# kevalmorabia97/CoVA-Web-Object-Detection

Measured on AMD Instinct MI355X. Metric: webpages/sec fwd+bwd (90 bboxes, K=24), higher is better.
Workload: dtype f32

## Files before the change

cova-web-object-detection_amd/csrc/bn1d.hip:

```cpp
#include "bn_tail.h"

namespace {

constexpr int COLS = 8, SLICES = 128, RUN = 32;
constexpr int THREADS = COLS * SLICES;

__device__ __forceinline__ void slices_total(double (*s_a)[COLS], double (*s_b)[COLS], int tx, int ty, double a, double b,
                                             double &ta, double &tb)
{
    s_a[ty][tx] = a;
    s_b[ty][tx] = b;
    __syncthreads();
    ta = 0.0;
    tb = 0.0;
    if (ty == 0)
        for (int j = 0; j < SLICES; ++j) {
            ta += s_a[j][tx];
            tb += s_b[j][tx];
        }
}

template <bool DROP>
__global__ __launch_bounds__(THREADS) void bn1d_fwd_kernel(
    const float *__restrict__ x, int ldx, int R, int C, const float *__restrict__ gamma, const float *__restrict__ beta,
// ... 213 lines not shown
    const float *__restrict__ invstd, const float *__restrict__ scale, int R, int C, float *__restrict__ dgamma,
    float *__restrict__ dbeta, float *__restrict__ dz, int lddz, float *__restrict__ dz_colsum)
{
    __shared__ double s_red[V4_THREADS / 64][V4_COLS][2];
    __shared__ float s_c1[V4_COLS], s_c2[V4_COLS];
    const int q = threadIdx.x & 1, slice = threadIdx.x >> 1, lane = threadIdx.x & 63, wave = threadIdx.x >> 6;
    const int c = blockIdx.x * V4_COLS + q * 4;
    const bool colok = c < C;
    const float inv = DROP ? 1.f / (1.f - p) : 1.f;
    float mu[4] = {0.f, 0.f, 0.f, 0.f}, is[4] = {0.f, 0.f, 0.f, 0.f}, sc[4] = {0.f, 0.f, 0.f, 0.f};
    if (colok) {
#pragma unroll
        for (int j = 0; j < 4; ++j) { mu[j] = mean[c + j]; is[j] = invstd[c + j]; sc[j] = scale[c + j]; }
    }
    float4 gv[NR], av[NR], zv[NR];
    uchar4 mv[NR];
#pragma unroll
    for (int u = 0; u < NR; ++u) {
        const int r = slice + u * V4_SLICES;
        const bool ok = colok && r < R;
        const size_t rr = ok ? (size_t)r : 0;
        const int cc = ok ? c : 0;
        gv[u] = *reinterpret_cast<const float4 *>(dout + rr * ldg + cc);
        zv[u] = *reinterpret_cast<const float4 *>(z + rr * ldz + cc);
        if (act != nullptr) av[u] = *reinterpret_cast<const float4 *>(act + rr * lda + cc);
        if (DROP) mv[u] = *reinterpret_cast<const uchar4 *>(drop_mask + rr * C + cc);
        if (!ok) gv[u] = make_float4(0.f, 0.f, 0.f, 0.f);
    }
    double v[4][2] = {{0.0, 0.0}, {0.0, 0.0}, {0.0, 0.0}, {0.0, 0.0}};
    float dy[NR][4], xh[NR][4];
#pragma unroll
    for (int u = 0; u < NR; ++u) {
        const float g4[4] = {gv[u].x, gv[u].y, gv[u].z, gv[u].w};
        const float z4[4] = {zv[u].x, zv[u].y, zv[u].z, zv[u].w};
        const float a4[4] = {av[u].x, av[u].y, av[u].z, av[u].w};
        const uint8_t m4[4] = {mv[u].x, mv[u].y, mv[u].z, mv[u].w};
#pragma unroll
        for (int j = 0; j < 4; ++j) {
            float g = g4[j];
            if (DROP) g = m4[j] ? g * inv : 0.f;
            if (act != nullptr && !(a4[j] > 0.f)) g = 0.f;
            dy[u][j] = g;
            xh[u][j] = (z4[j] - mu[j]) * is[j];
            v[j][0] += (double)g;
            v[j][1] = fma((double)g, (double)xh[u][j], v[j][1]);
        }
    }
    double ta, tb;
    v4_totals(s_red, v, q, lane, wave, ta, tb);
    const int cf = blockIdx.x * V4_COLS + threadIdx.x;
    if (threadIdx.x < V4_COLS && cf < C) {
        if (dbeta) dbeta[cf] = (float)ta;
        if (dgamma) dgamma[cf] = (float)tb;
        s_c1[threadIdx.x] = (float)(ta / (double)R);
        s_c2[threadIdx.x] = (float)(tb / (double)R);
    }
    __syncthreads();
    double cs[4][2] = {{0.0, 0.0}, {0.0, 0.0}, {0.0, 0.0}, {0.0, 0.0}};
    if (colok) {
        float s[4] = {0.f, 0.f, 0.f, 0.f};
#pragma unroll
        for (int u = 0; u < NR; ++u) {
            const int r = slice + u * V4_SLICES;
            if (r >= R) break;
            float o[4];
#pragma unroll
            for (int j = 0; j < 4; ++j) {
                o[j] = sc[j] * (dy[u][j] - s_c1[q * 4 + j] - xh[u][j] * s_c2[q * 4 + j]);
                s[j] += o[j];
            }
            *reinterpret_cast<float4 *>(dz + (size_t)r * lddz + c) = make_float4(o[0], o[1], o[2], o[3]);
        }
#pragma unroll
        for (int j = 0; j < 4; ++j) cs[j][0] = (double)s[j];
    }
    if (dz_colsum != nullptr) {
        __syncthreads();
        double t1, t2;
        v4_totals(s_red, cs, q, lane, wave, t1, t2);
        if (threadIdx.x < V4_COLS && cf < C) dz_colsum[cf] = (float)t1;
    }
}

int g_bn1d_variant = 1;

inline bool al16(const void *p) { return ((uintptr_t)p & 15) == 0; }

}

int cova_internal_set_bn1d_variant(int v) { g_bn1d_variant = v; return COVA_OK; }
int cova_internal_get_bn1d_variant() { return (int)g_bn1d_variant; }

COVA_API int cova_bn1d_fwd(const float *x, int ldx, int R, int C, const float *gamma, const float *beta,
                           float *running_mean, float *running_var, long long *num_batches_tracked, float momentum,
                           float eps, int relu, float *out, int ldo, float *dropped, int ld_dropped, uint8_t *mask,
                           float p, unsigned long long seed, int mask_given, float *scale, float *shift, float *mean,
                           float *invstd, void *stream)
{
    COVA_REQUIRE(x && gamma && beta && out && scale && shift && mean && invstd && R > 0 && C > 0);
    COVA_REQUIRE((running_mean == nullptr) == (running_var == nullptr));
    COVA_REQUIRE(dropped == nullptr || (mask != nullptr && p >= 0.f && p < 1.f));
    const bool v4 = g_bn1d_variant != 0 && C % 4 == 0 && ldx % 4 == 0 && ldo % 4 == 0 && al16(x) && al16(out) &&
                    (dropped == nullptr || (ld_dropped % 4 == 0 && al16(dropped) && ((uintptr_t)mask & 3) == 0)) &&
                    R <= 8 * V4_SLICES;
    if (v4) {
        const dim3 g4(cdiv(C, V4_COLS));
#define BN1D_FWD_V4(NR_, DROP_)                                                                                             \
        hipLaunchKernelGGL((bn1d_fwd_v4_kernel<NR_, DROP_>), g4, dim3(V4_THREADS), 0, (hipStream_t)stream, x, ldx, R, C, gamma, \
                           beta, running_mean, running_var, num_batches_tracked, momentum, eps, relu, out, ldo, dropped,   \
                           ld_dropped, mask, p, seed, mask_given, scale, shift, mean, invstd)
        if (R <= 3 * V4_SLICES) { if (dropped) BN1D_FWD_V4(3, true); else BN1D_FWD_V4(3, false); }
        else if (R <= 6 * V4_SLICES) { if (dropped) BN1D_FWD_V4(6, true); else BN1D_FWD_V4(6, false); }
        else { if (dropped) BN1D_FWD_V4(8, true); else BN1D_FWD_V4(8, false); }
#undef BN1D_FWD_V4
        COVA_LAUNCH_CHECK();
        return COVA_OK;
    }
    const dim3 grid(cdiv(C, COLS));
    if (dropped)
        hipLaunchKernelGGL(bn1d_fwd_kernel<true>, grid, dim3(THREADS), 0, (hipStream_t)stream, x, ldx, R, C, gamma, beta,
                           running_mean, running_var, num_batches_tracked, momentum, eps, relu, out, ldo, dropped,
                           ld_dropped, mask, p, seed, mask_given, scale, shift, mean, invstd);
    else
        hipLaunchKernelGGL(bn1d_fwd_kernel<false>, grid, dim3(THREADS), 0, (hipStream_t)stream, x, ldx, R, C, gamma, beta,
                           running_mean, running_var, num_batches_tracked, momentum, eps, relu, out, ldo, dropped,
                           ld_dropped, mask, p, seed, mask_given, scale, shift, mean, invstd);
    COVA_LAUNCH_CHECK();
    return COVA_OK;
}

COVA_API int cova_bn1d_bwd(const float *dout, int ldg, const uint8_t *drop_mask, float p, const float *act, int lda,
                           const float *z, int ldz, const float *mean, const float *invstd, const float *scale, int R,
                           int C, float *dgamma, float *dbeta, float *dz, int lddz, float *dz_colsum, void *stream)
{
    COVA_REQUIRE(dout && z && mean && invstd && scale && dz && R > 0 && C > 0);
    COVA_REQUIRE(drop_mask == nullptr || (p >= 0.f && p < 1.f));
    const bool v4 = g_bn1d_variant != 0 && C % 4 == 0 && ldg % 4 == 0 && ldz % 4 == 0 && lddz % 4 == 0 && al16(dout) &&
                    al16(z) && al16(dz) && (act == nullptr || (lda % 4 == 0 && al16(act))) &&
                    (drop_mask == nullptr || ((uintptr_t)drop_mask & 3) == 0) && R <= 6 * V4_SLICES;
    if (v4) {
        const dim3 g4(cdiv(C, V4_COLS));
#define BN1D_BWD_V4(NR_, DROP_)                                                                                             \
        hipLaunchKernelGGL((bn1d_bwd_v4_kernel<NR_, DROP_>), g4, dim3(V4_THREADS), 0, (hipStream_t)stream, dout, ldg, drop_mask, \
                           p, act, lda, z, ldz, mean, invstd, scale, R, C, dgamma, dbeta, dz, lddz, dz_colsum)
        if (R <= 3 * V4_SLICES) { if (drop_mask) BN1D_BWD_V4(3, true); else BN1D_BWD_V4(3, false); }
        else { if (drop_mask) BN1D_BWD_V4(6, true); else BN1D_BWD_V4(6, false); }
#undef BN1D_BWD_V4
        COVA_LAUNCH_CHECK();
        return COVA_OK;
    }
    const dim3 grid(cdiv(C, COLS));
    if (drop_mask)
        hipLaunchKernelGGL(bn1d_bwd_kernel<true>, grid, dim3(THREADS), 0, (hipStream_t)stream, dout, ldg, drop_mask, p, act,
                           lda, z, ldz, mean, invstd, scale, R, C, dgamma, dbeta, dz, lddz, dz_colsum);
    else
        hipLaunchKernelGGL(bn1d_bwd_kernel<false>, grid, dim3(THREADS), 0, (hipStream_t)stream, dout, ldg, drop_mask, p, act,
                           lda, z, ldz, mean, invstd, scale, R, C, dgamma, dbeta, dz, lddz, dz_colsum);
    COVA_LAUNCH_CHECK();
    return COVA_OK;
}
```

cova-web-object-detection_amd/engine.py:

```python
import ctypes
import os

import torch

from . import _lib
from .weights import BACKBONE_CHANNELS as C64

GAT_MAX_K = 1024

call, query = _lib.call, _lib.query
BN_MOMENTUM, BN_EPS, LEAKY_SLOPE = 0.1, 1e-5, 0.2


DROPOUT_KEYS = ("decoder.0", "decoder.3")


def is_train(training, key):
    if isinstance(training, bool):
        return training
    if hasattr(training, "get"):
        return bool(training.get(key, True))
    return bool(training)


# ... 212 lines not shown
    st = bn_state(C, like, count, training)
    g, b = params[prefix + "weight"], params[prefix + "bias"]
    rm, rv = buffers[prefix + "running_mean"], buffers[prefix + "running_var"]
    if training:
        upd = update_running
        partial, nparts = fold_partials(partial, nparts, 2 * C)
        if STAT_SYNC is not None:
            partial, nparts, count = _global_stats(partial, nparts, 2 * C, count, unit)
            st.count = float(count)
        nbt = buffers.get(prefix + "num_batches_tracked") if upd else None
        call("cova_bn_finalize_fwd", partial, nparts, C, float(count), g, b, rm if upd else None,
             rv if upd else None, nbt, BN_MOMENTUM, BN_EPS, st.scale, st.shift, st.mean, st.invstd)
    else:
        call("cova_bn_eval_params", g, b, rm, rv, BN_EPS, C, st.scale, st.shift, st.mean, st.invstd)
    return st


def colstats(x, ld, R, C):
    n = query("cova_colreduce_num_chunks", R, C)
    part = _empty((n, 2, C), x)
    call("cova_colstats", x, ld, R, C, part)
    return part, n


def bn_backward(dout, ldd, act, lda, z, ldz, st, R, dz, lddz, dres=None, lddres=0, gout=None,
                prefix=None, unit="boxes", drop=None, colsum=None):
    C = st.C
    if (bn1d_fused(not st.frozen) and dres is None and R > 0 and z.dim() == 2 and dz.data_ptr() != dout.data_ptr()):
        dgamma = _gbuf(gout, (prefix or "") + "weight", (C,), z)
        dbeta = _gbuf(gout, (prefix or "") + "bias", (C,), z)
        call("cova_bn1d_bwd", dout, ldd, drop[0] if drop else None, float(drop[1]) if drop else 0.0, act, lda, z, ldz,
             st.mean, st.invstd, st.scale, R, C, dgamma, dbeta, dz, lddz, colsum)
        return dgamma, dbeta
    if drop is not None:
        dy = _empty((R, C), dout)
        call("cova_dropout_bwd", dout, ldd, drop[0], dy, C, R, C, float(drop[1]))
        dout, ldd = dy, C
    n = query("cova_colreduce_num_chunks", R, C)
    part = _empty((n, 2, C), z)
    call("cova_bn_bwd_reduce", dout, ldd, act, lda, z, ldz, st.mean, st.invstd, R, C, part)
    dgamma = _gbuf(gout, (prefix or "") + "weight", (C,), z)
    dbeta = _gbuf(gout, (prefix or "") + "bias", (C,), z)
    coef = bn_finalize_bwd(part, n, C, R, dgamma, dbeta, unit, frozen=st.frozen)
    call("cova_bn_bwd_apply", dout, ldd, act, lda, z, ldz, st.mean, st.invstd, st.scale, coef, dz,
         lddz, dres, lddres, R, C)
    if colsum is not None:
        call("cova_colsum", dz, lddz, R, C, colsum)
    return dgamma, dbeta


class _BnTailStruct(ctypes.Structure):
    _fields_ = [("mode", ctypes.c_int), ("counter", ctypes.c_void_p), ("count", ctypes.c_double),
                ("gamma", ctypes.c_void_p), ("beta", ctypes.c_void_p), ("running_mean", ctypes.c_void_p),
                ("running_var", ctypes.c_void_p), ("num_batches_tracked", ctypes.c_void_p),
                ("momentum", ctypes.c_float), ("eps", ctypes.c_float), ("scale", ctypes.c_void_p),
                ("shift", ctypes.c_void_p), ("mean", ctypes.c_void_p), ("invstd", ctypes.c_void_p),
                ("dgamma", ctypes.c_void_p), ("dbeta", ctypes.c_void_p), ("abc", ctypes.c_void_p)]


class BnTail:
    _COUNTERS = {}

    def __init__(self, mode, like, count, **ptrs):
        key = (like.device, torch.cuda.current_stream(like.device).cuda_stream)
        ctr = BnTail._COUNTERS.get(key)
        if ctr is None:
            ctr = BnTail._COUNTERS[key] = torch.zeros((1,), dtype=torch.int32, device=like.device)
        self.keep = [ctr] + [v for v in ptrs.values() if isinstance(v, torch.Tensor)]
        c = _BnTailStruct()
        c.mode, c.counter, c.count = mode, ctr.data_ptr(), float(count)
        c.momentum, c.eps = BN_MOMENTUM, BN_EPS
        for k, v in ptrs.items():
            setattr(c, k, v.data_ptr() if isinstance(v, torch.Tensor) else None)
        self.c = c

    @property
    def ptr(self):
        return ctypes.addressof(self.c)


class Options:
    overlap_allreduce = os.environ.get("COVA_OVERLAP_ALLREDUCE", "1") != "0"
    bn_tail = os.environ.get("COVA_BN_TAIL", "1") != "0"


OPTIONS = Options()

CONV3_KEYS = ["convnet.4.0.conv1", "convnet.4.0.conv2", "convnet.4.1.conv1", "convnet.4.1.conv2"]
BN3_KEYS = ["convnet.4.0.bn1.", "convnet.4.0.bn2.", "convnet.4.1.bn1.", "convnet.4.1.bn2."]


class LazyFeature:
    __slots__ = ("z", "x", "scale", "shift", "shape")

    def __init__(self, z, x, scale, shift):
        self.z, self.x, self.scale, self.shift, self.shape = z, x, scale, shift, tuple(z.shape)


def is_bottleneck(params):
    return "convnet.4.0.conv3.weight" in params


@on_device_of(0)
def convstack_fwd(images, params, buffers, training, save=True, lazy_out=False):
    _check(images)
    B, _, H, W = images.shape
    H1, W1 = query("cova_conv_out_size", H, 7, 2, 3), query("cova_conv_out_size", W, 7, 2, 3)
    H2, W2 = query("cova_conv_out_size", H1, 3, 2, 1), query("cova_conv_out_size", W1, 3, 2, 1)
    bottleneck = is_bottleneck(params)
    layer2 = has_layer2(params)
    lazy_out = lazy_out and not layer2
    sv = {"images": images, "dims": (B, H, W, H1, W1, H2, W2), "kind": "bottleneck" if bottleneck else "basic"}
    if bottleneck:
        sv["_w3"] = conv3_weights([params["convnet.4.%d.conv2.weight" % b] for b in (0, 1, 2)], images)
    else:
        sv["_w3"] = conv3_weights([params[k + ".weight"] for k in CONV3_KEYS], images)
    y1 = _empty((B, H1, W1, C64), images)
    nt1 = query("cova_conv1_num_partials", B, H, W)
    stem_train = is_train(training, "convnet.1.")
    part = _empty((nt1, 2, C64), images) if stem_train else None
    if stem_train and tails_on():
        bn1, tail = bn_tail_fwd("convnet.1.", params, buffers, C64, images, B * H1 * W1)
        call("cova_conv1_fwd_tail", images, params["convnet.0.weight"], y1, part, B, H, W, tail.ptr)
    else:
        call("cova_conv1_fwd_tail", images, params["convnet.0.weight"], y1, part, B, H, W, None)
        bn1 = bn_params("convnet.1.", params, buffers, C64, images, training, part, nt1, B * H1 * W1, unit="pages")
    p1 = _empty((B, H2, W2, C64), images)
    idx = _empty((B, H2, W2, C64), images, torch.uint8)
    want_ymax = save and (stem_train or bottleneck)
    ymax = _empty((B, H2, W2, C64), images) if want_ymax else None
    call("cova_bn_relu_maxpool_fwd", y1, bn1.scale, bn1.shift, p1, idx, ymax, B, H1, W1)
    sv.update(y1=y1, bn1=bn1, idx=idx, ymax=ymax)
    if bottleneck:
        feat = _layer1_bottleneck_fwd(p1, params, buffers, training, save, lazy_out, sv)
    else:
        feat = _layer1_basic_fwd(p1, params, buffers, training, save, lazy_out, sv)
    if layer2:
        feat = _layer2_fwd(feat, params, buffers, training, save, sv)
    return feat, (sv if save else None)


def conv3_num_partials(B, H, W):
    return query("cova_conv3x3_wino4_num_partials", B, H, W)


def conv3x3_pro(u, inp, in2, abc, relu, addend, act, msc, msh, z, mean, invstd, out, part, B, H, W, tail=None,
                act_bits=None):
    if tail is not None:
        if act_bits is not None:
            act = None
        call("cova_conv3x3_wino4_full_tail", inp, in2, abc, relu, u, addend, act, act_bits, msc, msh, z, mean, invstd,
             out, part, B, H, W, tail.ptr)
    else:
        call("cova_conv3x3_wino4_full", inp, in2, abc, relu, u, addend, act, msc, msh, z, mean, invstd, out, part,
             B, H, W)


def conv3_weights(ws, like):
    n = len(ws)
    uf, ud = _empty((n, query("cova_conv3x3_wino4_u_floats")), like), _empty((n, query("cova_conv3x3_wino4_u_floats")), like)
    call("cova_conv3x3_wino4_prep_multi", *(list(ws) + [None] * (4 - n)), uf, ud)
    return [uf[i] for i in range(n)], [ud[i] for i in range(n)]


def conv_bn_fwd(u, inp, abc, relu, out, prefix, params, buffers, training, part, nt, R, B, H, W):
    training = is_train(training, prefix)
# ... 577 lines not shown
    N = bboxes.shape[0]
    PH, PW = roi_size
    call("cova_roialign_fwd", feat, bboxes, N, B, C, Hf, Wf, PH, PW, float(spatial_scale), int(sampling_ratio),
         1 if aligned else 0, out, ld_out)
    return dict(kind="align", bboxes=bboxes, shape=(B, Hf, Wf, C), roi=(PH, PW), scale=float(spatial_scale),
                sampling_ratio=int(sampling_ratio), aligned=bool(aligned), zmax=None)


def roialign_bwd(sv, gout, ld_g):
    B, Hf, Wf, C = sv["shape"]
    PH, PW = sv["roi"]
    gfeat = _empty((B, Hf, Wf, C), gout)
    call("cova_roialign_bwd", gout, ld_g, sv["bboxes"], sv["bboxes"].shape[0], B, C, Hf, Wf, PH, PW, sv["scale"],
         sv["sampling_ratio"], 1 if sv["aligned"] else 0, gfeat, _empty((2 * B + 16,), gout, torch.int32))
    return gfeat


def _roipool_ws(sv, like):
    B, Hf, Wf, C = sv["shape"]
    PH, PW = sv["roi"]
    return _empty((query("cova_roipool_bwd_workspace_words", sv["bboxes"].shape[0], B, C, PH, PW),), like, torch.int32)


def roipool_bwd(sv, gout, ld_g):
    B, Hf, Wf, C = sv["shape"]
    PH, PW = sv["roi"]
    gfeat = _empty((B, Hf, Wf, C), gout)
    call("cova_roipool_bwd", gout, ld_g, sv["bboxes"], sv["argmax"], sv["bboxes"].shape[0], B, C, Hf,
         Wf, PH, PW, float(sv["scale"]), gfeat, _roipool_ws(sv, gout))
    return gfeat


def roipool_bwd_bn(sv, gout, ld_g, last, grad_out=None):
    B, Hf, Wf, C = sv["shape"]
    PH, PW = sv["roi"]
    n = sv["bboxes"].shape[0]
    gfeat = _empty((B, Hf, Wf, C), gout)
    npart = query("cova_roipool_bwd_bn_num_partials", n)
    part = _empty((npart, 2, C), gout)
    bn = last["bn"]
    if tails_on(C) and not bn.frozen and last.get("prefix"):
        dg, db, abc, tail = bn_tail_bwd(bn, B * Hf * Wf, grad_out, last["prefix"], gout)
        call("cova_roipool_bwd_bn_tail", gout, ld_g, sv["pooled"], sv["ld_pooled"], sv["zmax"], sv["bboxes"],
             sv["argmax"], n, B, C, Hf, Wf, PH, PW, float(sv["scale"]), bn.mean, bn.invstd, gfeat, part,
             _roipool_ws(sv, gout), tail.ptr)
        return gfeat, {"pend": (dg, db, abc)}
    call("cova_roipool_bwd_bn", gout, ld_g, sv["pooled"], sv["ld_pooled"], sv["zmax"], sv["bboxes"], sv["argmax"],
         n, B, C, Hf, Wf, PH, PW, float(sv["scale"]), bn.mean, bn.invstd, gfeat, part, _roipool_ws(sv, gout))
    return gfeat, (part, npart)


def bn1d_fused(training):
    return OPTIONS.bn_tail and training and STAT_SYNC is None


def bn1d_fwd(x, ldx, N, C, prefix, params, buffers, training, out, ldo, relu, drop=None):
    training = is_train(training, prefix)
    if bn1d_fused(training) and N > 0:
        st = bn_state(C, x, N, True)
        dropped = mask = None
        p, seed, given = 0.0, 0, False
        if drop is not None:
            p, seed, mask = drop
            given = mask is not None
            if given:
                _check(mask, torch.uint8)
            else:
                mask = _empty((N, C), x, torch.uint8)
            dropped = _empty((N, C), x)
        call("cova_bn1d_fwd", x, ldx, N, C, params[prefix + "weight"], params[prefix + "bias"],
             buffers[prefix + "running_mean"], buffers[prefix + "running_var"],
             buffers.get(prefix + "num_batches_tracked"), BN_MOMENTUM, BN_EPS, 1 if relu else 0, out, ldo, dropped, C,
             mask, float(p), int(seed), 1 if given else 0, st.scale, st.shift, st.mean, st.invstd)
        return (st, dropped, mask) if drop is not None else st
    part, n = colstats(x, ldx, N, C) if training else (None, 0)
    st = bn_params(prefix, params, buffers, C, x, training, part, n, N)
    call("cova_bn_act_fwd", x, ldx, st.scale, st.shift, None, 0, out, ldo, N, C, 1 if relu else 0)
    if drop is not None:
        dropped, mask = dropout_fwd(out, ldo, N, C, drop[0], drop[1], drop[2])
        return st, dropped, mask
    return st


def bbox_fwd(bboxes, params, buffers, training, out, ldo):
    N = bboxes.shape[0]
    Hd = params["bbox_feat_encoder.0.weight"].shape[0]
    raw, z = _empty((N, 5), bboxes), _empty((N, Hd), bboxes)
    call("cova_bbox_linear_fwd", bboxes, params["bbox_feat_encoder.0.weight"],
         params["bbox_feat_encoder.0.bias"], raw, z, N, Hd)
    st = bn1d_fwd(z, Hd, N, Hd, "bbox_feat_encoder.1.", params, buffers, training, out, ldo, True)
    return dict(raw=raw, z=z, st=st, N=N, Hd=Hd, out=out, ldo=ldo)


def bbox_bwd(sv, g, ldg, gout=None):
    N, Hd = sv["N"], sv["Hd"]
    dz = _empty((N, Hd), g)
    dg, db = bn_backward(g, ldg, sv["out"], sv["ldo"], sv["z"], Hd, sv["st"], N, dz, Hd, None, 0,
                         gout, "bbox_feat_encoder.1.")
    dW = _gbuf(gout, "bbox_feat_encoder.0.weight", (Hd, 5), g)
    dbias = _gbuf(gout, "bbox_feat_encoder.0.bias", (Hd,), g)
    call("cova_bbox_linear_bwd", dz, sv["raw"], dW, dbias, N, Hd)
    return {"bbox_feat_encoder.0.weight": dW, "bbox_feat_encoder.0.bias": dbias,
            "bbox_feat_encoder.1.weight": dg, "bbox_feat_encoder.1.bias": db}


def _adjacent(a, b):
    return (a.is_contiguous() and b.is_contiguous() and a.shape[1:] == b.shape[1:] and
            b.data_ptr() == a.data_ptr() + a.numel() * a.element_size() and
            a.untyped_storage().data_ptr() == b.untyped_storage().data_ptr())


def edge_geometry(bboxes, ctx, page_size):
    _check(bboxes)
    _check(ctx, torch.int64)
    try:
        H, W = (float(v) for v in page_size)
    except (TypeError, ValueError):
        raise ValueError("page_size must be (height, width) in pixels, got %r" % (page_size,))
    if not (H > 0 and W > 0):
        raise ValueError("page_size must be positive, got %r" % (page_size,))
    N, K = ctx.shape
    phi = _empty((N, K, 8), bboxes)
    call("cova_edge_geometry", bboxes, ctx, N, K, W, H, phi)
    return phi


def gat_fwd(h, ldh, N, F, ctx, params, hprime, ldo, prefix="gat.", phi=None):
    _check(ctx, torch.int64)
    Wi, Wj = params[prefix + "W_i.weight"], params[prefix + "W_j.weight"]
    aw, ab = params[prefix + "attention_layer.weight"], params[prefix + "attention_layer.bias"]
    ew = params.get(prefix + "edge_layer.weight")
    if (ew is None) != (phi is None):
        raise ValueError("%s: %s" % (prefix, "an edge-aware head needs the edge features phi (boxes and page size)"
                                     if phi is None else "edge features given to a head without edge_layer.weight"))
    D, K = Wi.shape[0], ctx.shape[1]
    Wh = _empty((N, 2 * D), h)
    if _adjacent(Wi, Wj):
        call("cova_sgemm", 0, 1, N, 2 * D, F, h, ldh, Wi, F, Wh, 2 * D, None, 0)
    else:
        call("cova_sgemm", 0, 1, N, D, F, h, ldh, Wi, F, Wh, 2 * D, None, 0)
        call("cova_sgemm", 0, 1, N, D, F, h, ldh, Wj, F, Wh[:, D:], 2 * D, None, 0)
    s, t, attn = _empty((N,), h), _empty((N,), h), _empty((N, K), h)
    if phi is None:
        call("cova_gat_fwd", Wh, 2 * D, aw, ab, ctx, N, K, D, LEAKY_SLOPE, s, t, attn, hprime, ldo)
    else:
        assert tuple(phi.shape) == (N, K, 8), (tuple(phi.shape), N, K)
        call("cova_gat_fwd_edge", Wh, 2 * D, aw, ab, ctx, _check(phi), _check(ew), N, K, D, LEAKY_SLOPE, s, t, attn,
             hprime, ldo)
    return dict(h=h, ldh=ldh, N=N, F=F, D=D, K=K, ctx=ctx, Wh=Wh, s=s, t=t, attn=attn, prefix=prefix, phi=phi)


_CSR_WS = {}


def gat_transpose(ctx):
    N, K = ctx.shape
    key = (ctx.device, torch.cuda.current_stream(ctx.device).cuda_stream, N, K)
    csr = _CSR_WS.get(key)
    if csr is None:
        if len(_CSR_WS) >= 8:
            _CSR_WS.clear()
        csr = _CSR_WS[key] = torch.zeros((query("cova_gat_transpose_ints", N, K),), dtype=torch.int32, device=ctx.device)
    try:
        call("cova_gat_transpose_reuse", ctx, N, K, csr)
    except BaseException:
        _CSR_WS.pop(key, None)
        raise
    return csr


def gat_bwd(sv, g, ldg, params, dh, lddh, accumulate_dh, gout=None, csr=None):
    N, F, D, K, prefix = sv["N"], sv["F"], sv["D"], sv["K"], sv["prefix"]
    if csr is None:
        csr = gat_transpose(sv["ctx"])
    du = _empty((N, K), g)
    Wi, Wj = params[prefix + "W_i.weight"], params[prefix + "W_j.weight"]
    aw = params[prefix + "attention_layer.weight"]
    dWh = _empty((N, 2 * D), g)
# ... 312 lines not shown
```

include/cova_hip.h:

```cpp
#ifndef COVA_HIP_H
#define COVA_HIP_H

#include <stdint.h>

#ifdef __cplusplus
extern "C" {
#endif

#define COVA_ERR_BAD_ARG 10001

typedef struct cova_bn_tail {
    int mode;
    int *counter;
    double count;
    const float *gamma, *beta;
    float *running_mean, *running_var;
    long long *num_batches_tracked;
    float momentum, eps;
    float *scale, *shift, *mean, *invstd;
    float *dgamma, *dbeta, *abc;
} cova_bn_tail;

int cova_conv_out_size(int in_size, int kernel, int stride, int pad);
int cova_set_option(int key, int value);
// ... 110 lines not shown
                         float momentum, float eps, float *scale, float *shift, float *mean,
                         float *invstd, void *stream);
int cova_bn_eval_params(const float *gamma, const float *beta, const float *running_mean,
                        const float *running_var, float eps, int C, float *scale, float *shift,
                        float *mean , float *invstd , void *stream);
int cova_bn_act_fwd(const float *z, int ldz, const float *scale, const float *shift,
                    const float *res , int ldres, float *out, int ldo, long long R, int C,
                    int relu, void *stream);
int cova_bn_act_fwd_bits(const float *z, const float *scale, const float *shift, const float *res, float *out,
                         uint32_t *bits, long long R, void *stream);
int cova_bn_act2_fwd(const float *z, const float *scale, const float *shift, const float *z2,
                     const float *scale2, const float *shift2, float *out, long long R, int C, int relu,
                     void *stream);
int cova_bn_bwd_reduce(const float *dout, int ldd, const float *act ,
                       int lda, const float *z, int ldz, const float *mean, const float *invstd,
                       long long R, int C, float *partial , void *stream);
int cova_bn_finalize_bwd(const float *partial, int nparts, int C, double count,
                         float *dgamma , float *dbeta , float *coef ,
                         void *stream);
int cova_bn_finalize_bwd_abc(const float *partial, int nparts, int C, double count,
                             float *dgamma , float *dbeta , const float *mean,
                             const float *invstd, const float *scale, float *abc, void *stream);
int cova_bn_bwd_apply(const float *dout, int ldd, const float *act, int lda, const float *z, int ldz,
                      const float *mean, const float *invstd, const float *scale, const float *coef,
                      float *dz, int lddz, float *dres , int lddres, long long R, int C,
                      void *stream);
int cova_bn1d_fwd(const float *x, int ldx, int R, int C, const float *gamma, const float *beta,
                  float *running_mean , float *running_var, long long *num_batches_tracked ,
                  float momentum, float eps, int relu, float *out, int ldo, float *dropped , int ld_dropped,
                  uint8_t *mask, float p, unsigned long long seed, int mask_given, float *scale, float *shift,
                  float *mean, float *invstd, void *stream);
int cova_bn1d_bwd(const float *dout, int ldg, const uint8_t *drop_mask , float p,
                  const float *act , int lda, const float *z, int ldz, const float *mean,
                  const float *invstd, const float *scale, int R, int C, float *dgamma, float *dbeta, float *dz,
                  int lddz, float *dz_colsum , void *stream);
int cova_bn_relu_maxpool_fwd(const float *y , const float *scale, const float *shift,
                             float *out , uint8_t *idx,
                             float *ymax , int B, int H1,
                             int W1, void *stream);
int cova_bn_relu_maxpool_bwd_num_partials(int B, int H1, int W1);
int cova_bn_relu_maxpool_bwd_reduce(const float *dp, const uint8_t *idx, const float *y,
                                    const float *scale, const float *shift, const float *mean,
                                    const float *invstd, float *partial, int B, int H1, int W1,
                                    void *stream);
int cova_bn_relu_maxpool_bwd_apply(const float *dp, const uint8_t *idx, const float *y,
                                   const float *scale, const float *shift, const float *mean,
                                   const float *invstd, const float *coef, float *dz, int B, int H1,
                                   int W1, void *stream);

int cova_roipool_fwd(const float *feat, const float *rois, int n_rois, int B, int C, int H, int W,
                     int PH, int PW, float spatial_scale, float *out, int ld_out, int32_t *argmax,
                     void *stream);
int cova_roipool_bwd(const float *gout, int ld_g, const float *rois, const int32_t *argmax,
                     int n_rois, int B, int C, int H, int W, int PH, int PW, float spatial_scale,
                     float *gfeat, void *ws , void *stream);
int cova_roipool_bwd_workspace_words(int n_rois, int B, int C, int PH, int PW);
int cova_roipool_bwd_bn_num_partials(int n_rois);
int cova_roipool_bwd_bn(const float *gout, int ld_g, const float *pooled, int ld_p, const float *zmax,
                        const float *rois, const int32_t *argmax, int n_rois, int B, int C, int H, int W,
                        int PH, int PW, float spatial_scale, const float *mean, const float *invstd,
                        float *gfeat, float *partial, void *ws ,
                        void *stream);
int cova_roipool_bwd_bn_tail(const float *gout, int ld_g, const float *pooled, int ld_p, const float *zmax,
                             const float *rois, const int32_t *argmax, int n_rois, int B, int C, int H, int W,
                             int PH, int PW, float spatial_scale, const float *mean, const float *invstd,
                             float *gfeat, float *partial, void *ws, const cova_bn_tail *tail, void *stream);
int cova_roipool_fwd_bn(const float *z, const float *x, const float *scale, const float *shift,
                        const float *rois, int n_rois, int B, int C, int H, int W, int PH, int PW,
                        float spatial_scale, float *out, int ld_out, int32_t *argmax,
                        float *zmax ,
                        void *stream);

int cova_roialign_fwd(const float *feat, const float *rois, int n_rois, int B, int C, int H, int W, int PH,
                      int PW, float spatial_scale, int sampling_ratio, int aligned, float *out, int ld_out,
                      void *stream);
int cova_roialign_bwd(const float *gout, int ld_g, const float *rois, int n_rois, int B, int C, int H, int W,
                      int PH, int PW, float spatial_scale, int sampling_ratio, int aligned, float *gfeat,
                      void *ws, void *stream);

int cova_bbox_linear_fwd(const float *bboxes, const float *W , const float *bias,
                         float *raw , float *z , int N, int Hd, void *stream);
int cova_bbox_linear_bwd(const float *dz, const float *raw, float *dW, float *db, int N, int Hd,
                         void *stream);

int cova_sgemm(int transA, int transB, int M, int N, int K, const float *A, int lda, const float *B,
               int ldb, float *C, int ldc, const float *bias , int accumulate,
               void *stream);
int cova_sgemm_dropout_bwd(int transA, int transB, int M, int N, int K, const float *A, int lda, const float *B,
                           int ldb, float *C, int ldc, const uint8_t *keep , float p, void *stream);

int cova_gat_fwd(const float *Wh, int ldw, const float *att_w , const float *att_b ,
                 const int64_t *ctx , int N, int K, int D, float slope, float *s ,
                 float *t , float *attn , float *hprime, int ldh, void *stream);
int cova_gat_transpose_ints(int N, int K);
int cova_gat_transpose(const int64_t *ctx, int N, int K, int *csr , void *stream);
int cova_gat_transpose_reuse(const int64_t *ctx, int N, int K, int *csr, void *stream);
int cova_gat_bwd(const float *g, int ldg, const float *Wh, int ldw, const float *s, const float *t,
                 const float *attn, const int64_t *ctx, const float *att_w, int N, int K, int D,
                 float slope, float *dWh , int lddw, float *ds , float *dt ,
                 float *d_att_w , float *d_att_b , const int *csr ,
                 float *du , void *stream);
int cova_gat_fwd_edge(const float *Wh, int ldw, const float *att_w , const float *att_b ,
                      const int64_t *ctx , const float *phi , const float *edge_w , int N,
                      int K, int D, float slope, float *s , float *t , float *attn ,
                      float *hprime, int ldh, void *stream);
int cova_gat_edge_workspace_floats(int N, int K);
int cova_gat_bwd_edge(const float *g, int ldg, const float *Wh, int ldw, const float *s, const float *t,
                      const float *attn, const int64_t *ctx, const float *att_w, const float *phi ,
                      const float *edge_w , int N, int K, int D, float slope, float *dWh , int lddw,
                      float *ds , float *dt , float *d_att_w , float *d_att_b ,
                      float *d_edge_w , const int *csr, float *du , float *workspace, void *stream);

int cova_dropout_fwd(const float *x, int ldx, float *out, int ldo, uint8_t *mask ,
                     long long R, int C, float p, unsigned long long seed, int mask_given,
                     void *stream);
int cova_dropout_bwd(const float *g, int ldg, const uint8_t *mask, float *dx, int ldx, long long R,
                     int C, float p, void *stream);
int cova_linear_small_fwd(const float *x, int ldx, const float *W , const float *b,
                          float *y , int N, int Cin, int NC, void *stream);
int cova_linear_small_bwd(const float *dy, const float *x, int ldx, const float *W, float *dx,
                          int lddx, float *dW, float *db, int N, int Cin, int NC, void *stream);
int cova_ce_sum(const float *logits, const int64_t *labels , int N, int NC, float gscale,
                float *loss , float *dlogits , int64_t *pred ,
                void *stream);
int cova_adam_step(float *p, const float *g, float *m, float *v, long long n, int step, double lr,
                   double beta1, double beta2, double eps, double weight_decay, void *stream);
int cova_colsum(const float *x, int ldx, int R, int C, float *out, void *stream);

int cova_optim_step(int algo, float *p, const float *g, float *m, float *v, long long n, const long long *segs, int n_seg,
                    long long total, const double *groups, int n_groups, int step, const float *gscale, void *stream);
int cova_grad_norm_workspace_doubles(long long total);
int cova_grad_norm(const float *g, long long n, const long long *segs, int n_seg, long long total, double max_norm,
                   double *workspace, float *out, void *stream);
int cova_ce_loss_workspace_doubles(int N);
int cova_ce_loss_fwd(const float *logits, const int64_t *labels, int N, int NC, const float *class_weight ,
                     double label_smoothing, double focal_gamma, long long ignore_index, int has_ignore_index,
                     double *acc, int64_t *pred , int64_t *metrics , double *workspace,
                     void *stream);
int cova_ce_loss_bwd(const float *logits, const int64_t *labels, int N, int NC, const float *class_weight ,
                     double label_smoothing, double focal_gamma, long long ignore_index, int has_ignore_index,
                     const double *acc_total, int reduction_mean, const float *grad_scale ,
                     float *loss_out , float *dlogits , void *stream);
int cova_page_class_topk(const float *logits, const int64_t *page_start, int n_pages, int NC, int k,
                         int64_t *out, void *stream);
int cova_eval_page_ranks(const float *logits, const int64_t *labels, const int64_t *page_start,
                         const int *page_ids , int B, int NC, int P, int *rank,
                         int *top1 , void *stream);

int cova_images_u8_to_f32(const uint8_t *u8_nhwc, float *f32_nchw, int B, int H, int W, void *stream);
int cova_collate_boxes(const float *rows, const int *page_offsets, int B, int N, int context_size,
                       float *bboxes, long long *labels, long long *ctx ,
                       void *stream);
int cova_pages_u8_gather_f32(const uint8_t *store_u8, const int *page_idx, int P, int B, int H, int W, float *f32_nchw,
                             void *stream);
int cova_sample_boxes_workspace_ints(int B, int N);
int cova_sample_boxes(const float *rows, const int *page_offsets, const int *row_starts ,
                      const int *page_ids , const int *keep_counts, int B, int N,
                      const long long *keys , unsigned long long stream_seed, int *workspace, int *sel,
                      int *out_offsets, void *stream);
int cova_collate_selected(const float *rows, const int *sel, const int *out_offsets, int B, int N_out, int context_size,
                          float *bboxes, long long *labels, long long *ctx ,
                          const float *addl_in , int A, float *addl_out ,
                          void *stream);
int cova_context_knn(const float *bboxes, const int *page_offsets, int B, int N, int context_size, int k_spatial,
                     long long *ctx, void *stream);
int cova_edge_geometry(const float *bboxes, const long long *ctx, int N, int K, float img_w, float img_h, float *phi,
// ... 12 lines not shown
```

Baseline: 1764.

## Fuse bbox linear encoder with BatchNorm1d+ReLU in forward and backward kernels

Adds a single kernel that computes the bbox feature linear layer, batch statistics, BN normalization and ReLU in one launch for small row counts. A second kernel fuses the BN backward with the bbox linear weight and bias gradient reduction through shared memory, so the dz buffer is never written to global memory. This removes several small kernel launches and intermediate round trips per step. It is limited to N at most 3*V4_SLICES and Hd divisible by 4, and it keeps a strict FMA ordering to match the reference numerics.

```diff
diff --git a/cova-web-object-detection_amd/csrc/bn1d.hip b/cova-web-object-detection_amd/csrc/bn1d.hip
--- a/cova-web-object-detection_amd/csrc/bn1d.hip
+++ b/cova-web-object-detection_amd/csrc/bn1d.hip
@@ -319,6 +319,186 @@
     }
 }
 
+constexpr int BB_NR = 3, BB_MAX_ROWS = BB_NR * V4_SLICES;
+constexpr int BB_PARTS = 256, BB_PSTRIDE = BB_PARTS + 1;
+
+__device__ __forceinline__ float bbox_linear_out(const float (&f)[5], const float *__restrict__ w, float b)
+{
+#pragma clang fp contract(off)
+    float acc = fmaf(f[0], w[0], 0.f);
+#pragma unroll
+    for (int k = 1; k < 5; ++k) {
+        const float p = f[k] * w[k];
+        acc = acc + p;
+    }
+    return acc + b;
+}
+
+__global__ __launch_bounds__(V4_THREADS) void bbox_bn1d_fwd_kernel(
+    const float *__restrict__ bboxes, const float *__restrict__ Wt , const float *__restrict__ bias,
+    float *__restrict__ raw , float *__restrict__ z , int R, int C, const float *__restrict__ gamma,
+    const float *__restrict__ beta, float *__restrict__ running_mean, float *__restrict__ running_var,
+    long long *__restrict__ nbt, float momentum, float eps, float *__restrict__ out, int ldo, float *__restrict__ scale,
+    float *__restrict__ shift, float *__restrict__ mean, float *__restrict__ invstd)
+{
+    __shared__ double s_red[V4_THREADS / 64][V4_COLS][2];
+    __shared__ float s_sc[V4_COLS], s_sh[V4_COLS];
+    const int q = threadIdx.x & 1, slice = threadIdx.x >> 1, lane = threadIdx.x & 63, wave = threadIdx.x >> 6;
+    const int c = blockIdx.x * V4_COLS + q * 4;
+    const bool colok = c < C;
+    float4 xv[BB_NR];
+    double v[4][2] = {{0.0, 0.0}, {0.0, 0.0}, {0.0, 0.0}, {0.0, 0.0}};
+#pragma unroll
+    for (int u = 0; u < BB_NR; ++u) {
+        const int r = slice + u * V4_SLICES;
+        xv[u] = make_float4(0.f, 0.f, 0.f, 0.f);
+        if (colok && r < R) {
+            const float *bb = bboxes + 5 * r;
+            const float x1 = bb[1], y1 = bb[2];
+            const float w = bb[3] - x1, h = bb[4] - y1;
+            const float f[5] = {x1, y1, w, h, w / h};
+            if (c == 0) {
+#pragma unroll
+                for (int k = 0; k < 5; ++k) raw[5 * r + k] = f[k];
+            }
+            float zz[4];
+#pragma unroll
+            for (int j = 0; j < 4; ++j) zz[j] = bbox_linear_out(f, Wt + (c + j) * 5, bias[c + j]);
+            xv[u] = make_float4(zz[0], zz[1], zz[2], zz[3]);
+            *reinterpret_cast<float4 *>(z + (size_t)r * C + c) = xv[u];
+        }
+    }
+#pragma unroll
+    for (int u = 0; u < BB_NR; ++u) {
+        const double d[4] = {(double)xv[u].x, (double)xv[u].y, (double)xv[u].z, (double)xv[u].w};
+#pragma unroll
+        for (int j = 0; j < 4; ++j) {
+            v[j][0] += d[j];
+            v[j][1] = fma(d[j], d[j], v[j][1]);
+        }
+    }
+    double ta, tb;
+    v4_totals(s_red, v, q, lane, wave, ta, tb);
+    const int cf = blockIdx.x * V4_COLS + threadIdx.x;
+    if (threadIdx.x < V4_COLS && cf < C) {
+        bn_fwd_channel(ta, tb, (double)R, cf, gamma, beta, running_mean, running_var, momentum, eps, scale, shift, mean,
+                       invstd);
+        s_sc[threadIdx.x] = scale[cf];
+        s_sh[threadIdx.x] = shift[cf];
+    }
+    if (blockIdx.x == 0 && threadIdx.x == 0 && nbt != nullptr) *nbt += 1;
+    __syncthreads();
+    if (!colok) return;
+    const float sc[4] = {s_sc[q * 4], s_sc[q * 4 + 1], s_sc[q * 4 + 2], s_sc[q * 4 + 3]};
+    const float sh[4] = {s_sh[q * 4], s_sh[q * 4 + 1], s_sh[q * 4 + 2], s_sh[q * 4 + 3]};
+#pragma unroll
+    for (int u = 0; u < BB_NR; ++u) {
+        const int r = slice + u * V4_SLICES;
+        if (r >= R) break;
+        const float xs[4] = {xv[u].x, xv[u].y, xv[u].z, xv[u].w};
+        float y[4];
+#pragma unroll
+        for (int j = 0; j < 4; ++j) {
+            y[j] = fmaf(sc[j], xs[j], sh[j]);
+            y[j] = y[j] > 0.f ? y[j] : 0.f;
+        }
+        *reinterpret_cast<float4 *>(out + (size_t)r * ldo + c) = make_float4(y[0], y[1], y[2], y[3]);
+    }
+}
+
+__global__ __launch_bounds__(V4_THREADS) void bbox_bn1d_bwd_kernel(
+    const float *__restrict__ dout, int ldg, const float *__restrict__ act, int lda, const float *__restrict__ z,
+    const float *__restrict__ mean, const float *__restrict__ invstd, const float *__restrict__ scale,
+    const float *__restrict__ raw, int R, int C, float *__restrict__ dgamma, float *__restrict__ dbeta,
+    float *__restrict__ dW , float *__restrict__ db )
+{
+    __shared__ double s_red[V4_THREADS / 64][V4_COLS][2];
+    __shared__ float s_c1[V4_COLS], s_c2[V4_COLS];
+    __shared__ __align__(16) float s_buf[BB_MAX_ROWS * V4_COLS > V4_COLS * 6 * BB_PSTRIDE ? BB_MAX_ROWS * V4_COLS : V4_COLS * 6 * BB_PSTRIDE];
+    const int q = threadIdx.x & 1, slice = threadIdx.x >> 1, lane = threadIdx.x & 63, wave = threadIdx.x >> 6;
+    const int c = blockIdx.x * V4_COLS + q * 4;
+    const bool colok = c < C;
+    float mu[4] = {0.f, 0.f, 0.f, 0.f}, is[4] = {0.f, 0.f, 0.f, 0.f}, sc[4] = {0.f, 0.f, 0.f, 0.f};
+    if (colok) {
+#pragma unroll
+        for (int j = 0; j < 4; ++j) { mu[j] = mean[c + j]; is[j] = invstd[c + j]; sc[j] = scale[c + j]; }
+    }
+    float4 gv[BB_NR], av[BB_NR], zv[BB_NR];
+#pragma unroll
+    for (int u = 0; u < BB_NR; ++u) {
+        const int r = slice + u * V4_SLICES;
+        const bool ok = colok && r < R;
+        const size_t rr = ok ? (size_t)r : 0;
+        const int cc = ok ? c : 0;
+        gv[u] = *reinterpret_cast<const float4 *>(dout + rr * ldg + cc);
+        zv[u] = *reinterpret_cast<const float4 *>(z + rr * C + cc);
+        av[u] = *reinterpret_cast<const float4 *>(act + rr * lda + cc);
+        if (!ok) gv[u] = make_float4(0.f, 0.f, 0.f, 0.f);
+    }
+    double v[4][2] = {{0.0, 0.0}, {0.0, 0.0}, {0.0, 0.0}, {0.0, 0.0}};
+    float dy[BB_NR][4], xh[BB_NR][4];
+#pragma unroll
+    for (int u = 0; u < BB_NR; ++u) {
+        const float g4[4] = {gv[u].x, gv[u].y, gv[u].z, gv[u].w};
+        const float z4[4] = {zv[u].x, zv[u].y, zv[u].z, zv[u].w};
+        const float a4[4] = {av[u].x, av[u].y, av[u].z, av[u].w};
+#pragma unroll
+        for (int j = 0; j < 4; ++j) {
+            float g = g4[j];
+            if (!(a4[j] > 0.f)) g = 0.f;
+            dy[u][j] = g;
+            xh[u][j] = (z4[j] - mu[j]) * is[j];
+            v[j][0] += (double)g;
+            v[j][1] = fma((double)g, (double)xh[u][j], v[j][1]);
+        }
+    }
+    double ta, tb;
+    v4_totals(s_red, v, q, lane, wave, ta, tb);
+    const int cf = blockIdx.x * V4_COLS + threadIdx.x;
+    if (threadIdx.x < V4_COLS && cf < C) {
+        if (dbeta) dbeta[cf] = (float)ta;
+        if (dgamma) dgamma[cf] = (float)tb;
+        s_c1[threadIdx.x] = (float)(ta / (double)R);
+        s_c2[threadIdx.x] = (float)(tb / (double)R);
+    }
+    __syncthreads();
+#pragma unroll
+    for (int u = 0; u < BB_NR; ++u) {
+        const int r = slice + u * V4_SLICES;
+        if (r >= R) break;
+        float o[4];
+#pragma unroll
+        for (int j = 0; j < 4; ++j) o[j] = sc[j] * (dy[u][j] - s_c1[q * 4 + j] - xh[u][j] * s_c2[q * 4 + j]);
+        *reinterpret_cast<float4 *>(s_buf + r * V4_COLS + q * 4) = make_float4(o[0], o[1], o[2], o[3]);
+    }
+    __syncthreads();
+    const int col = threadIdx.x & (V4_COLS - 1), t0 = threadIdx.x / V4_COLS;
+    float a[2][6] = {{0, 0, 0, 0, 0, 0}, {0, 0, 0, 0, 0, 0}};
+#pragma unroll
+    for (int i = 0; i < 2; ++i)
+        for (int n = t0 + i * (V4_THREADS / V4_COLS); n < R; n += BB_PARTS) {
+            const float g = s_buf[n * V4_COLS + col];
+#pragma unroll
+            for (int k = 0; k < 5; ++k) a[i][k] += g * raw[5 * n + k];
+            a[i][5] += g;
+        }
+    __syncthreads();
+#pragma unroll
+    for (int i = 0; i < 2; ++i)
+#pragma unroll
+        for (int k = 0; k < 6; ++k) s_buf[(col * 6 + k) * BB_PSTRIDE + t0 + i * (V4_THREADS / V4_COLS)] = a[i][k];
+    __syncthreads();
+    if (threadIdx.x < V4_COLS * 6) {
+        const int jc = threadIdx.x / 6, k = threadIdx.x - jc * 6, j = blockIdx.x * V4_COLS + jc;
+        float t = 0.f;
+        for (int i = 0; i < BB_PARTS; ++i) t += s_buf[(jc * 6 + k) * BB_PSTRIDE + i];
+        if (j < C) {
+            if (k < 5) dW[j * 5 + k] = t;
+            else db[j] = t;
+        }
+    }
+}
+
 int g_bn1d_variant = 1;
 
 inline bool al16(const void *p) { return ((uintptr_t)p & 15) == 0; }
@@ -396,3 +576,33 @@
     COVA_LAUNCH_CHECK();
     return COVA_OK;
 }
+
+COVA_API int cova_bbox_bn1d_max_rows(int Hd) { return g_bn1d_variant != 0 && Hd > 0 && Hd % 4 == 0 ? BB_MAX_ROWS : 0; }
+
+COVA_API int cova_bbox_bn1d_fwd(const float *bboxes, const float *W, const float *bias, float *raw, float *z, int N, int Hd,
+                                const float *gamma, const float *beta, float *running_mean, float *running_var,
+                                long long *num_batches_tracked, float momentum, float eps, float *out, int ldo,
+                                float *scale, float *shift, float *mean, float *invstd, void *stream)
+{
+    COVA_REQUIRE(bboxes && W && bias && raw && z && gamma && beta && out && scale && shift && mean && invstd);
+    COVA_REQUIRE((running_mean == nullptr) == (running_var == nullptr));
+    COVA_REQUIRE(N > 0 && N <= cova_bbox_bn1d_max_rows(Hd) && ldo % 4 == 0 && al16(z) && al16(out));
+    hipLaunchKernelGGL(bbox_bn1d_fwd_kernel, dim3(cdiv(Hd, V4_COLS)), dim3(V4_THREADS), 0, (hipStream_t)stream, bboxes, W,
+                       bias, raw, z, N, Hd, gamma, beta, running_mean, running_var, num_batches_tracked, momentum, eps, out,
+                       ldo, scale, shift, mean, invstd);
+    COVA_LAUNCH_CHECK();
+    return COVA_OK;
+}
+
+COVA_API int cova_bbox_bn1d_bwd(const float *dout, int ldg, const float *act, int lda, const float *z, const float *raw,
+                                const float *mean, const float *invstd, const float *scale, int N, int Hd, float *dgamma,
+                                float *dbeta, float *dW, float *db, void *stream)
+{
+    COVA_REQUIRE(dout && act && z && raw && mean && invstd && scale && dW && db);
+    COVA_REQUIRE(N > 0 && N <= cova_bbox_bn1d_max_rows(Hd) && ldg % 4 == 0 && lda % 4 == 0 && al16(dout) && al16(act) &&
+                 al16(z));
+    hipLaunchKernelGGL(bbox_bn1d_bwd_kernel, dim3(cdiv(Hd, V4_COLS)), dim3(V4_THREADS), 0, (hipStream_t)stream, dout, ldg, act,
+                       lda, z, mean, invstd, scale, raw, N, Hd, dgamma, dbeta, dW, db);
+    COVA_LAUNCH_CHECK();
+    return COVA_OK;
+}
diff --git a/cova-web-object-detection_amd/engine.py b/cova-web-object-detection_amd/engine.py
--- a/cova-web-object-detection_amd/engine.py
+++ b/cova-web-object-detection_amd/engine.py
@@ -318,6 +318,7 @@
 class Options:
     overlap_allreduce = os.environ.get("COVA_OVERLAP_ALLREDUCE", "1") != "0"
     bn_tail = os.environ.get("COVA_BN_TAIL", "1") != "0"
+    head_fused = os.environ.get("COVA_HEAD_FUSED", "1") != "0"
 
 
 OPTIONS = Options()
@@ -1061,18 +1062,40 @@
     return st
 
 
+def bbox_fused(N, Hd, training, *operands):
+    return (OPTIONS.head_fused and bn1d_fused(training) and 0 < N <= query("cova_bbox_bn1d_max_rows", Hd) and
+            all(t.data_ptr() % 16 == 0 and ld % 4 == 0 for t, ld in zip(operands[::2], operands[1::2])))
+
+
 def bbox_fwd(bboxes, params, buffers, training, out, ldo):
     N = bboxes.shape[0]
     Hd = params["bbox_feat_encoder.0.weight"].shape[0]
     raw, z = _empty((N, 5), bboxes), _empty((N, Hd), bboxes)
+    prefix = "bbox_feat_encoder.1."
+    if bbox_fused(N, Hd, is_train(training, prefix), out, ldo):
+        st = bn_state(Hd, z, N, True)
+        call("cova_bbox_bn1d_fwd", bboxes, params["bbox_feat_encoder.0.weight"], params["bbox_feat_encoder.0.bias"], raw, z,
+             N, Hd, params[prefix + "weight"], params[prefix + "bias"], buffers[prefix + "running_mean"],
+             buffers[prefix + "running_var"], buffers.get(prefix + "num_batches_tracked"), BN_MOMENTUM, BN_EPS, out, ldo,
+             st.scale, st.shift, st.mean, st.invstd)
+        return dict(raw=raw, z=z, st=st, N=N, Hd=Hd, out=out, ldo=ldo)
     call("cova_bbox_linear_fwd", bboxes, params["bbox_feat_encoder.0.weight"],
          params["bbox_feat_encoder.0.bias"], raw, z, N, Hd)
-    st = bn1d_fwd(z, Hd, N, Hd, "bbox_feat_encoder.1.", params, buffers, training, out, ldo, True)
+    st = bn1d_fwd(z, Hd, N, Hd, prefix, params, buffers, training, out, ldo, True)
     return dict(raw=raw, z=z, st=st, N=N, Hd=Hd, out=out, ldo=ldo)
 
 
 def bbox_bwd(sv, g, ldg, gout=None):
     N, Hd = sv["N"], sv["Hd"]
+    if bbox_fused(N, Hd, not sv["st"].frozen, g, ldg, sv["out"], sv["ldo"]):
+        st, prefix = sv["st"], "bbox_feat_encoder.1."
+        dg, db = _gbuf(gout, prefix + "weight", (Hd,), g), _gbuf(gout, prefix + "bias", (Hd,), g)
+        dW = _gbuf(gout, "bbox_feat_encoder.0.weight", (Hd, 5), g)
+        dbias = _gbuf(gout, "bbox_feat_encoder.0.bias", (Hd,), g)
+        call("cova_bbox_bn1d_bwd", g, ldg, sv["out"], sv["ldo"], sv["z"], sv["raw"], st.mean, st.invstd, st.scale, N, Hd,
+             dg, db, dW, dbias)
+        return {"bbox_feat_encoder.0.weight": dW, "bbox_feat_encoder.0.bias": dbias,
+                "bbox_feat_encoder.1.weight": dg, "bbox_feat_encoder.1.bias": db}
     dz = _empty((N, Hd), g)
     dg, db = bn_backward(g, ldg, sv["out"], sv["ldo"], sv["z"], Hd, sv["st"], N, dz, Hd, None, 0,
                          gout, "bbox_feat_encoder.1.")
diff --git a/include/cova_hip.h b/include/cova_hip.h
--- a/include/cova_hip.h
+++ b/include/cova_hip.h
@@ -216,6 +216,16 @@
                          float *raw , float *z , int N, int Hd, void *stream);
 int cova_bbox_linear_bwd(const float *dz, const float *raw, float *dW, float *db, int N, int Hd,
                          void *stream);
+int cova_bbox_bn1d_max_rows(int Hd);
+int cova_bbox_bn1d_fwd(const float *bboxes, const float *W , const float *bias, float *raw ,
+                       float *z , int N, int Hd, const float *gamma, const float *beta,
+                       float *running_mean , float *running_var, long long *num_batches_tracked ,
+                       float momentum, float eps, float *out, int ldo, float *scale, float *shift, float *mean,
+                       float *invstd, void *stream);
+int cova_bbox_bn1d_bwd(const float *dout, int ldg, const float *act, int lda, const float *z ,
+                       const float *raw , const float *mean, const float *invstd, const float *scale, int N,
+                       int Hd, float *dgamma , float *dbeta , float *dW ,
+                       float *db , void *stream);
 
 int cova_sgemm(int transA, int transB, int M, int N, int K, const float *A, int lda, const float *B,
                int ldb, float *C, int ldc, const float *bias , int accumulate,
```

Result: slower. 1732 (-1.8%).
